# underdoc-wang/ST-MGCN

Hardware: AMD Instinct MI355X
Metric: train_samples_per_sec (higher is better)
Workload: dtype bf16; 1 GPU; model=ST_MGCN, preset=bench-1024, n_nodes=1024, seq_len=8, m_graphs=3, lstm_hidden=64, gcn_hidden=64, global_batch=32, parallelism=dp1, hipgraph=True, impl=hip

## Files before the change

### stmgcn_amd/csrc/fused_rnn.hip

```cpp

#include "common.h"

#define RNN_H 64
static_assert(4 * RNN_H == STM_DA_GATES, "dA tile layout assumes 4H = 256");
#define MAX_LAYERS 8
#define MAX_T 16

struct RnnPtrs {
  const void* w_ih[MAX_LAYERS];
  const void* w_hh[MAX_LAYERS];
  const void* b_ih[MAX_LAYERS];
  const void* b_hh[MAX_LAYERS];
};


extern "C" __global__ void mfma_probe_kernel(const __hip_bfloat16* A,
                                             const __hip_bfloat16* B, float* D) {
  const int l = threadIdx.x;
  bf16x8 a, b;
  #pragma unroll
      for (int j = 0; j < 8; ++j) {
    a[j] = *(const __bf16*)&A[(l % 16) * 32 + (l / 16) * 8 + j];
    b[j] = *(const __bf16*)&B[((l / 16) * 8 + j) * 16 + (l % 16)];
  }
  f32x4 c = {0.f, 0.f, 0.f, 0.f};
  c = mfma16x16x32(a, b, c);
  #pragma unroll
      for (int r = 0; r < 4; ++r) D[((l / 16) * 4 + r) * 16 + (l % 16)] = c[r];
}

template <typename F> __device__ __forceinline__ void rnn_uniform_bool(bool flag, F&& f) {
  if (flag) f(std::true_type{});
  else f(std::false_type{});
}

template <typename T, bool CIN1, bool GRU>
__global__ void __launch_bounds__(256, 2)
lstm_fwd_kernel(const T* __restrict__ x,
                T* __restrict__ out,
                T* __restrict__ hseq_g,
                T* __restrict__ cseq_g,
                T* __restrict__ gates_g,
                RnnPtrs ptrs,
                int S, int Tst, int L, int ret_seq) {
  using frag = typename Frag8<T>::type;
  using elem = typename Frag8<T>::elem;
  typedef elem elem4 __attribute__((ext_vector_type(4)));
  constexpr int MT = SEQ_TILE / 16;
  constexpr int SLOT = SEQ_TILE * 128;
  extern __shared__ char lds[];
  const int s0 = blockIdx.x * SEQ_TILE;
  const int wv = threadIdx.x >> 6;
  const int lane = threadIdx.x & 63;
  const int l16 = lane & 15;
  const int lgrp = lane >> 4;
  const long S_pad = (long)gridDim.x * SEQ_TILE;

  auto hslot = [&](int par) -> char* { return lds + (par & 1) * SLOT; };
  char* xbuf = lds + 2 * SLOT;

  if (CIN1) {
    for (int i = threadIdx.x; i < SEQ_TILE * Tst; i += 256) {
      const int s = i % SEQ_TILE, t = i / SEQ_TILE;
      T v = fromF<T>(0.f);
      if (s0 + s < S) v = x[(long)(s0 + s) * Tst + t];
      ((T*)xbuf)[t * SEQ_TILE + s] = v;
    }
    __syncthreads();
  }

  const int hch = 16 * wv + l16;
  const unsigned wlane = (hch * RNN_H + lgrp * 8) * sizeof(T);
  const unsigned inlane = (l16 * RNN_H + lgrp * 8) * sizeof(T);
  const unsigned savelane = (wv * MT * 64 + lane) * sizeof(T);

  auto layer_body = [&](int layer, auto first_c, auto train_c, auto top_c) {
    constexpr bool FIRST = decltype(first_c)::value;
    constexpr bool TRAIN = decltype(train_c)::value;
    constexpr bool TOP = decltype(top_c)::value;
    constexpr bool SCALAR = CIN1 && FIRST;
    constexpr bool KEEP_H = TRAIN || !TOP;
    const char* Whh = (const char*)ptrs.w_hh[layer];
    const char* Wih = (const char*)ptrs.w_ih[layer];
    const T* bih = (const T*)ptrs.b_ih[layer];
    const T* bhh = (const T*)ptrs.b_hh[layer];

    const T* hin = FIRST ? nullptr
        : hseq_g + ((long)(layer - 1) * Tst) * (S_pad * RNN_H) + (long)s0 * RNN_H;

    frag xfr[MT][2];
    auto load_input = [&](int t) {
      #pragma unroll
      for (int m = 0; m < MT; ++m) {
        #pragma unroll
        for (int kk = 0; kk < 2; ++kk) {
          if constexpr (FIRST) {
            const char* xt = (const char*)(x + ((long)(s0 + 16 * m) * Tst + t) * RNN_H);
            const unsigned xlane = (l16 * Tst * RNN_H + lgrp * 8) * sizeof(T);
            xfr[m][kk] = frag{};
            if (s0 + 16 * m + l16 < S)
              xfr[m][kk] = *(const frag*)(xt + (xlane + kk * 32 * sizeof(T)));
          } else {
            const char* ht = (const char*)(hin + (long)t * (S_pad * RNN_H));
            xfr[m][kk] = *(const frag*)(ht + (inlane + (m * 16 * RNN_H + kk * 32) * sizeof(T)));
          }
        }
      }
    };
    if constexpr (!SCALAR) load_input(0);

    frag bhfrag[4][2];
    #pragma unroll
    for (int q = 0; q < 4; ++q)
      #pragma unroll
      for (int kk = 0; kk < 2; ++kk)
        bhfrag[q][kk] = *(const frag*)(Whh + (wlane + (q * 64 * RNN_H + kk * 32) * sizeof(T)));
    frag bxfrag[4][2];
    if constexpr (!SCALAR) {
      #pragma unroll
      for (int q = 0; q < 4; ++q)
        #pragma unroll
        for (int kk = 0; kk < 2; ++kk)
          bxfrag[q][kk] = *(const frag*)(Wih + (wlane + (q * 64 * RNN_H + kk * 32) * sizeof(T)));
    }
    float wih0[4];
    float bias[4];
    #pragma unroll
    for (int q = 0; q < 4; ++q) {
      const int g = q * 64 + hch;
      bias[q] = toF<T>(bih[g]) + toF<T>(bhh[g]);
      if constexpr (SCALAR) wih0[q] = toF<T>(((const T*)Wih)[g]);
    }

    float c_state[MT][4];
    #pragma unroll
    for (int m = 0; m < MT; ++m)
      #pragma unroll
      for (int r = 0; r < 4; ++r) c_state[m][r] = 0.f;

    #pragma clang loop unroll(disable)
    for (int t = 0; t < Tst; ++t) {
      f32x4 acc[MT][4];
      const f32x4 zero4 = {0.f, 0.f, 0.f, 0.f};

      if (t > 0) {
        char* slot = hslot(t - 1);
        #pragma unroll
        for (int m = 0; m < MT; ++m) {
          const int row = 16 * m + l16;
          #pragma unroll
          for (int kk = 0; kk < 2; ++kk) {
            frag a = *(const frag*)&slot[lds_swz(row, (kk * 32 + lgrp * 8) * 2)];
            #pragma unroll
            for (int q = 0; q < 4; ++q)
              acc[m][q] = mfma16x16x32(a, bhfrag[q][kk], kk == 0 ? zero4 : acc[m][q]);
          }
        }
      } else {
        asm volatile("");
        #pragma unroll
        for (int m = 0; m < MT; ++m)
          #pragma unroll
          for (int q = 0; q < 4; ++q) acc[m][q] = zero4;
      }
      if constexpr (!SCALAR) {
        #pragma unroll
        for (int m = 0; m < MT; ++m)
          #pragma unroll
          for (int kk = 0; kk < 2; ++kk)
            #pragma unroll
            for (int q = 0; q < 4; ++q)
              acc[m][q] = mfma16x16x32(xfr[m][kk], bxfrag[q][kk], acc[m][q]);
        if (t + 1 < Tst) load_input(t + 1);
      }

      constexpr bool GRU_FUSED_ZH = CIN1 && std::is_same<T, __half>::value;
      T hval[MT][4];
      frag gsave[MT][2];
      elem4 csave[MT];
      #pragma unroll
      for (int m = 0; m < MT; ++m) {
        float xv[4];
        if constexpr (SCALAR) {
          #pragma unroll
          for (int r = 0; r < 4; ++r)
            xv[r] = toF<T>(((const T*)xbuf)[t * SEQ_TILE + 16 * m + 4 * lgrp + r]);
        }
        #pragma unroll
        for (int r = 0; r < 4; ++r) {
          float pre[4];
          #pragma unroll
          for (int q = 0; q < 4; ++q) {
            pre[q] = stm_fadd(acc[m][q][r], bias[q]);
            if constexpr (SCALAR) pre[q] = stm_fadd(pre[q], stm_fmul(xv[r], wih0[q]));
          }
          const float gi = pre[0], gf = pre[1], gg = pre[2], go = pre[3];
          if constexpr (GRU) {
            const float r_ = stm_sigmoid(gi), z_ = stm_sigmoid(gf);
            const float n_ = stm_tanh(fmaf(r_, go, gg));
            const float hprev = c_state[m][r];
            csave[m][r] = (elem)hprev;
            const float zn = stm_fmul(1.f - z_, n_);
            const float h_ = GRU_FUSED_ZH ? fmaf(z_, hprev, zn)
                                          : fmaf(1.f - z_, n_, stm_fmul(z_, hprev));
            c_state[m][r] = h_;
            if constexpr (GRU_FUSED_ZH) {
              unsigned hw;
              asm("v_fma_mixlo_f16 %0, %1, %2, %3"
                  : "=v"(hw) : "v"(hprev), "v"(z_), "v"(zn));
              hval[m][r] = __builtin_bit_cast(T, (unsigned short)hw);
            } else {
              hval[m][r] = fromF<T>(h_);
            }
            gsave[m][0][0 + r] = (elem)r_;
            gsave[m][0][4 + r] = (elem)z_;
            gsave[m][1][0 + r] = (elem)n_;
            gsave[m][1][4 + r] = (elem)go;
          } else {
            const float i_ = stm_sigmoid(gi), f_ = stm_sigmoid(gf);
            const float g_ = stm_tanh(gg), o_ = stm_sigmoid(go);
            const float ig = stm_fmul(i_, g_);
            const float c_ = CIN1 ? stm_fadd(stm_fmul(f_, c_state[m][r]), ig)
                                  : fmaf(f_, c_state[m][r], ig);
            c_state[m][r] = c_;
            csave[m][r] = (elem)c_;
            const float h_ = stm_fmul(o_, stm_tanh(c_));
            hval[m][r] = fromF<T>(h_);
            gsave[m][0][0 + r] = (elem)i_;
            gsave[m][0][4 + r] = (elem)f_;
            gsave[m][1][0 + r] = (elem)g_;
            gsave[m][1][4 + r] = (elem)o_;
          }
        }
      }

      {
        char* slot = hslot(t);
        #pragma unroll
        for (int m = 0; m < MT; ++m)
          #pragma unroll
          for (int r = 0; r < 4; ++r) {
            const int row = 16 * m + 4 * lgrp + r;
            *(T*)&slot[lds_swz(row, hch * 2)] = hval[m][r];
          }
      }
      __syncthreads();

      {
        static_assert(SEQ_TILE * 8 == 256, "one 16 B piece of the slot per thread");
        const int c8 = threadIdx.x & 7, sr = threadIdx.x >> 3;
        const frag v = *(const frag*)&hslot(t)[lds_swz(sr, c8 * 16)];
        if constexpr (KEEP_H) {
          char* hp = (char*)(hseq_g + ((long)layer * Tst + t) * (S_pad * RNN_H)
                             + (long)s0 * RNN_H);
          *(frag*)(hp + threadIdx.x * 16) = v;
        }
        if constexpr (TOP) {
          if (s0 + sr < S) {
            if (ret_seq)
              *(frag*)&out[((long)(s0 + sr) * Tst + t) * RNN_H + c8 * 8] = v;
            else if (t == Tst - 1)
              *(frag*)&out[(long)(s0 + sr) * RNN_H + c8 * 8] = v;
          }
        }
      }

      if constexpr (TRAIN) {
        const long base = ((long)layer * Tst + t);
        char* gp = (char*)(gates_g + base * (S_pad * 4 * RNN_H)
                           + (long)blockIdx.x * (SEQ_TILE * 4 * RNN_H));
        #pragma unroll
        for (int m = 0; m < MT; ++m)
          #pragma unroll
          for (int hq = 0; hq < 2; ++hq)
            *(frag*)(gp + (savelane * 16 + (m * 64 * 16 + hq * 8) * sizeof(T))) = gsave[m][hq];
        char* cp = (char*)(cseq_g + base * (S_pad * RNN_H)
                           + (long)blockIdx.x * (SEQ_TILE * RNN_H));
        #pragma unroll
        for (int m = 0; m < MT; ++m)
          *(elem4*)(cp + (savelane * 4 + m * 64 * 4 * sizeof(T))) = csave[m];
      }
    }
  };

  for (int layer = 0; layer < L; ++layer) {
    rnn_uniform_bool(layer == 0, [&](auto first_c) {
      rnn_uniform_bool(gates_g != nullptr, [&](auto train_c) {
        rnn_uniform_bool(layer == L - 1, [&](auto top_c) {
          layer_body(layer, first_c, train_c, top_c);
        });
      });
    });
    __threadfence_block();
    __syncthreads();
  }
}

static RnnPtrs rnn_ptrs(int L, const void** w_ih, const void** w_hh,
                        const void** b_ih, const void** b_hh) {
  RnnPtrs p{};
  for (int l = 0; l < L && l < MAX_LAYERS; ++l) {
    p.w_ih[l] = w_ih[l]; p.w_hh[l] = w_hh[l];
    p.b_ih[l] = b_ih ? b_ih[l] : nullptr;
    p.b_hh[l] = b_hh ? b_hh[l] : nullptr;
  }
  return p;
}

template <typename F> void rnn_dispatch_variant(int cin, int gru, F&& f) {
  stm_dispatch_bool(cin == 1, [&](auto cin1) {
    stm_dispatch_bool(gru != 0, [&](auto is_gru) { f(cin1, is_gru); });
  });
}

extern "C" void stmgcn_lstm_fwd(void* stream, int dtype, const void* x,
                                void* out, void* hseq_g, void* cseq_g,
                                void* gates_g, const void** w_ih,
                                const void** w_hh, const void** b_ih,
                                const void** b_hh, int S, int Tst, int L,
                                int cin, int ret_seq, int gru) {
  const RnnPtrs p = rnn_ptrs(L, w_ih, w_hh, b_ih, b_hh);
  const int nblk = (S + SEQ_TILE - 1) / SEQ_TILE;
  stm_dispatch_lowp("stmgcn_lstm_fwd", dtype, [&](auto t) {
    using T = decltype(t);
    const size_t lds_bytes =
        2 * SEQ_TILE * 128 + (cin == 1 ? Tst * SEQ_TILE * sizeof(T) : 0);
    rnn_dispatch_variant(cin, gru, [&](auto cin1, auto is_gru) {
      hipLaunchKernelGGL(
          (lstm_fwd_kernel<T, decltype(cin1)::value, decltype(is_gru)::value>),
          dim3(nblk), dim3(256), lds_bytes, (hipStream_t)stream, (const T*)x,
          (T*)out, (T*)hseq_g, (T*)cseq_g, (T*)gates_g, p, S, Tst, L, ret_seq);
    });
  });
}

extern "C" void stmgcn_mfma_probe(void* stream_v, const void* A, const void* B,
                                  void* D) {
  hipLaunchKernelGGL(mfma_probe_kernel, dim3(1), dim3(64), 0,
                     (hipStream_t)stream_v, (const __hip_bfloat16*)A,
                     (const __hip_bfloat16*)B, (float*)D);
}


template <typename T> __device__ __forceinline__ unsigned long pack4_word(f32x4 v) {
  unsigned long w = 0;
  #pragma unroll
  for (int r = 0; r < 4; ++r)
    w |= (unsigned long)__builtin_bit_cast(unsigned short, fromF<T>(v[r])) << (16 * r);
  return w;
}

template <int CTRL> __device__ __forceinline__ float dpp_row_add(float v) {
  return v + __int_as_float(__builtin_amdgcn_update_dpp(
                 0, __float_as_int(v), CTRL, 0xf, 0xf, false));
}

__device__ __forceinline__ int swzA(int s, int cbyte) {
  return s * 512 + (cbyte ^ ((s & 15) << 4));
}

template <typename T, bool CIN1, bool GRU>
__global__ void __launch_bounds__(256, 2)
lstm_bwd_kernel(const T* __restrict__ dout,
                const T* __restrict__ x,
                const T* __restrict__ cseq_g,
                const T* __restrict__ gates_g,
                RnnPtrs w,
                T* __restrict__ dx,
                T* __restrict__ dA_g,
                T* __restrict__ dh_g,
                int S, int Tst, int L, int ret_seq) {
  using frag = typename Frag8<T>::type;
  using elem = typename Frag8<T>::elem;
  constexpr int MT = SEQ_TILE / 16;
  extern __shared__ char lds[];
  const int s0 = blockIdx.x * SEQ_TILE;
  const int wv = threadIdx.x >> 6;
  const int lane = threadIdx.x & 63;
  const int l16 = lane & 15;
  const int lgrp = lane >> 4;
  const long S_pad = (long)gridDim.x * SEQ_TILE;
  const int hch = 16 * wv + l16;

  char* dA_lds = lds;
  float* red = (float*)(dA_lds + SEQ_TILE * 512);
  char* gstage = (char*)(red + 4 * SEQ_TILE);
  char* dhstage = gstage + 256 * (MT * 32);
  char* cstage = dhstage + 256 * (MT * 8);
  char* wstage = cstage + 2 * 256 * (MT * 8);
  char* wmine = wstage + threadIdx.x * 16;

  for (int layer = L - 1; layer >= 0; --layer) {
    const bool l0cin1 = CIN1 && layer == 0;
    const T* WhhT = (const T*)w.w_hh[layer];
    const T* WihT = (const T*)w.w_ih[layer];
    float dh_rec[MT][4], dc[MT][4];
    #pragma unroll
    for (int m = 0; m < MT; ++m)
      #pragma unroll
      for (int r = 0; r < 4; ++r) { dh_rec[m][r] = 0.f; dc[m][r] = 0.f; }

    const long lay_base = (long)layer * Tst;
    auto lane_frag = [&](int m) -> unsigned { return (wv * MT + m) * 64 + lane; };
    auto g_at = [&](int t) {
      return gates_g + (lay_base + t) * (S_pad * 4 * RNN_H)
             + (long)blockIdx.x * (SEQ_TILE * 4 * RNN_H);
    };
    auto c_at = [&](int t) {
      return cseq_g + (lay_base + t) * (S_pad * RNN_H)
             + (long)blockIdx.x * (SEQ_TILE * RNN_H);
    };
    auto dh_at = [&](int t) {
      return dh_g + (long)t * (S_pad * RNN_H)
             + (long)blockIdx.x * (SEQ_TILE * RNN_H);
    };
    char* gmine = gstage + threadIdx.x * (MT * 32);
    #pragma unroll
    for (int m = 0; m < MT; ++m) {
      *(frag*)&gmine[m * 32 + 0] =
          *(((const frag*)(g_at(Tst - 1) + lane_frag(m) * 16)) + 0);
      *(frag*)&gmine[m * 32 + 16] =
          *(((const frag*)(g_at(Tst - 1) + lane_frag(m) * 16)) + 1);
    }
    ulong1* dhmine = (ulong1*)(dhstage + threadIdx.x * (MT * 8));
    auto cmine = [&](int t) {
      return (ulong1*)(cstage + ((t & 1) * 256 + threadIdx.x) * (MT * 8));
    };
    if (layer < L - 1) {
      #pragma unroll
      for (int m = 0; m < MT; ++m)
        dhmine[m] = *(const ulong1*)(dh_at(Tst - 1) + lane_frag(m) * 4);
    }
    #pragma unroll
    for (int m = 0; m < MT; ++m) {
      cmine(Tst - 1)[m] = *(const ulong1*)(c_at(Tst - 1) + lane_frag(m) * 4);
      if (!GRU && Tst >= 2)
        cmine(Tst - 2)[m] = *(const ulong1*)(c_at(Tst - 2) + lane_frag(m) * 4);
    }
    {
      const unsigned wl = (hch * (4 * RNN_H) + lgrp * 8) * sizeof(T);
      #pragma unroll
      for (int kk = 0; kk < 8; ++kk)
        *(frag*)&wmine[kk * 4096] = *(const frag*)((const char*)WhhT + (wl + kk * 64));
    }
    float wih0[4];
    if (l0cin1) {
      #pragma unroll
      for (int q = 0; q < 4; ++q) wih0[q] = toF<T>(WihT[q * 64 + hch]);
    }
    __threadfence_block();
    __syncthreads();

    unsigned long dh_sent[MT] = {};
    #pragma clang loop unroll(disable)
    for (int t = Tst - 1;; --t) {
      const long base = lay_base + t;

      float dxpart[MT][4];
      alignas(16) T pk[4][MT * 4];

      const bool top_dout = layer == L - 1 && (ret_seq || t == Tst - 1);
      T dov[MT][4];
      if (top_dout) {
        const int dstride = ret_seq ? Tst * RNN_H : RNN_H;
        const T* dtile = dout + (long)s0 * dstride + (ret_seq ? t * RNN_H : 0);
        const int last = S - 1 - s0;
        int row0 = 4 * lgrp;
        asm volatile("" : "+v"(row0));
        #pragma unroll
        for (int m = 0; m < MT; ++m)
          #pragma unroll
          for (int r = 0; r < 4; ++r) {
            const int row = 16 * m + row0 + r;
            dov[m][r] = dtile[(row < last ? row : last) * dstride + hch];
          }
      }

      #pragma unroll
      for (int m = 0; m < MT; ++m) {
        frag gf0 = *(const frag*)&gmine[m * 32 + 0];
        frag gf1 = *(const frag*)&gmine[m * 32 + 16];
        const ulong1 cc_t = cmine(t)[m];
        const ulong1 cc_p = (!GRU && t > 0) ? cmine(t - 1)[m] : ulong1{0};
        ulong1 dhup = ulong1{0};
        if (layer < L - 1) dhup = dhmine[m];
        f32x4 ct, cpv;
        #pragma unroll
        for (int r = 0; r < 4; ++r) {
          ct[r] = elemF(((const elem*)&cc_t)[r]);
          cpv[r] = elemF(((const elem*)&cc_p)[r]);
        }
        #pragma unroll
        for (int r = 0; r < 4; ++r) {
          const int row = 16 * m + 4 * lgrp + r;
          float dh = dh_rec[m][r];
          if (layer < L - 1) {
            dh += elemF(((const elem*)&dhup)[r]);
          } else if (top_dout) {
            dh = (s0 + row < S) ? dh + toF<T>(dov[m][r]) : dh;
          }
          float dAi, dAf, dAg, dAo;
          if (GRU) {
            const float r_ = elemF(gf0[r]);
            const float z_ = elemF(gf0[4 + r]);
            const float n_ = elemF(gf1[r]);
            const float Bn = elemF(gf1[4 + r]);
            const float hprev = ct[r];
            dh += dc[m][r];
            const float dz_pre = dh * (hprev - n_) * z_ * (1.f - z_);
            const float dn_pre = dh * (1.f - z_) * (1.f - n_ * n_);
            const float dBn = dn_pre * r_;
            const float dr_pre = dn_pre * Bn * r_ * (1.f - r_);
            dc[m][r] = dh * z_;
            dAi = dr_pre; dAf = dz_pre; dAg = dn_pre; dAo = dBn;
          } else {
            const float i_ = elemF(gf0[r]);
            const float f_ = elemF(gf0[4 + r]);
            const float g_ = elemF(gf1[r]);
            const float o_ = elemF(gf1[4 + r]);
            const float tc = stm_tanh(ct[r]);
            float dcv = dc[m][r] + dh * o_ * (1.f - tc * tc);
            dAo = dh * tc * o_ * (1.f - o_);
            dAi = dcv * g_ * i_ * (1.f - i_);
            dAf = dcv * cpv[r] * f_ * (1.f - f_);
            dAg = dcv * i_ * (1.f - g_ * g_);
            dc[m][r] = dcv * f_;
          }
          pk[0][4 * m + r] = fromF<T>(dAi);
          pk[1][4 * m + r] = fromF<T>(dAf);
          pk[2][4 * m + r] = fromF<T>(dAg);
          pk[3][4 * m + r] = fromF<T>(dAo);
          #pragma unroll
          for (int q = 0; q < 4; ++q)
            *(T*)&dA_lds[swzA(row, (q * 64 + hch) * 2)] = pk[q][4 * m + r];
          if (l0cin1)
            dxpart[m][r] = dAi * wih0[0] + dAf * wih0[1] + dAg * wih0[2] + dAo * wih0[3];
        }
      }
      if (l0cin1) {
        #pragma unroll
        for (int m = 0; m < MT; ++m)
          #pragma unroll
          for (int r = 0; r < 4; ++r) dxpart[m][r] = dpp_row_add<0xB1>(dxpart[m][r]);
        #pragma unroll
        for (int m = 0; m < MT; ++m)
          #pragma unroll
          for (int r = 0; r < 4; ++r) dxpart[m][r] = dpp_row_add<0x4E>(dxpart[m][r]);
        #pragma unroll
        for (int m = 0; m < MT; ++m)
          #pragma unroll
          for (int r = 0; r < 4; ++r) dxpart[m][r] = dpp_row_add<0x141>(dxpart[m][r]);
        #pragma unroll
        for (int m = 0; m < MT; ++m)
          #pragma unroll
          for (int r = 0; r < 4; ++r) {
            const float v = dpp_row_add<0x140>(dxpart[m][r]);
            if (l16 == 0) red[wv * SEQ_TILE + 16 * m + 4 * lgrp + r] = v;
          }
      }
      T* out_dA = dA_g + stm_da_tile_off(base * S_pad + s0);
      #pragma unroll
      for (int q = 0; q < 4; ++q) *(frag*)&gmine[q * 16] = *(const frag*)pk[q];
      auto stage_rest = [&](auto rec_c, auto inp_c, auto up_c) {
        constexpr bool REC = decltype(rec_c)::value;
        constexpr bool INP = decltype(inp_c)::value;
        constexpr bool UP = decltype(up_c)::value;
        const unsigned wlane = (hch * (4 * RNN_H) + lgrp * 8) * sizeof(T);
        frag b2[2][4];
        f32x4 acc1[MT], acc2[MT];
        #pragma unroll
        for (int m = 0; m < MT; ++m) {
          acc1[m] = f32x4{0.f, 0.f, 0.f, 0.f};
          acc2[m] = f32x4{0.f, 0.f, 0.f, 0.f};
        }
        auto mfma_half = [&](int h) {
          frag b1[4];
          if constexpr (REC) {
            #pragma unroll
            for (int j = 0; j < 4; ++j) b1[j] = *(const frag*)&wmine[(4 * h + j) * 4096];
          }
          if constexpr (REC || INP) {
            #pragma unroll
            for (int jb = 0; jb < 4; jb += 2) {
              frag a[2][MT];
              #pragma unroll
              for (int j = 0; j < 2; ++j)
                #pragma unroll
                for (int m = 0; m < MT; ++m)
                  a[j][m] = *(const frag*)&dA_lds[swzA(16 * m + l16, ((4 * h + jb + j) * 32 + lgrp * 8) * 2)];
              #pragma unroll
              for (int j = 0; j < 2; ++j)
                #pragma unroll
                for (int m = 0; m < MT; ++m) {
                  if constexpr (REC) acc1[m] = mfma16x16x32(a[j][m], b1[jb + j], acc1[m]);
                  if constexpr (INP) acc2[m] = mfma16x16x32(a[j][m], b2[h][jb + j], acc2[m]);
                }
            }
          }
        };
        if constexpr (INP) {
          #pragma unroll
          for (int m = 0; m < MT; ++m) asm volatile("" :: "v"(dh_sent[m]));
        }
        if constexpr (INP) {
          #pragma unroll
          for (int kk = 0; kk < 8; ++kk)
            b2[kk / 4][kk % 4] = *(const frag*)((const char*)WihT + (wlane + kk * 64));
        }
        ulong1 dhnext[MT], cnext[MT];
        frag gld[MT][2];
        if constexpr (REC) {
          __builtin_amdgcn_sched_barrier(0);
          #pragma unroll
          for (int m = 0; m < MT; ++m) {
            gld[m][0] = *(((const frag*)(g_at(t - 1) + lane_frag(m) * 16)) + 0);
            gld[m][1] = *(((const frag*)(g_at(t - 1) + lane_frag(m) * 16)) + 1);
          }
          const int tc = GRU ? t - 1 : (t >= 2 ? t - 2 : 0);
          #pragma unroll
          for (int m = 0; m < MT; ++m)
            cnext[m] = *(const ulong1*)(c_at(tc) + lane_frag(m) * 4);
          if constexpr (UP) {
            #pragma unroll
            for (int m = 0; m < MT; ++m)
              dhnext[m] = *(const ulong1*)(dh_at(t - 1) + lane_frag(m) * 4);
          }
          __builtin_amdgcn_sched_barrier(0);
        }
        #pragma unroll
        for (int q = 0; q < 4; ++q)
          *(frag*)&out_dA[(unsigned)stm_da_elem(q * RNN_H + hch, 8 * lgrp)] =
              *(const frag*)&gmine[q * 16];

        __builtin_amdgcn_sched_barrier(0);
        __syncthreads();
        mfma_half(0);
        mfma_half(1);
        if constexpr (REC) {
          #pragma unroll
          for (int m = 0; m < MT; ++m)
            #pragma unroll
            for (int r = 0; r < 4; ++r) dh_rec[m][r] = acc1[m][r];
        }

        if constexpr (INP) {
          if (layer > 0) {
            #pragma unroll
            for (int m = 0; m < MT; ++m) {
              dh_sent[m] = pack4_word<T>(acc2[m]);
              *(unsigned long*)(dh_at(t) + lane_frag(m) * 4) = dh_sent[m];
            }
          } else {
            T* dxtile = dx + ((long)s0 * Tst + t) * RNN_H;
            const unsigned dxlane = 4 * lgrp * (Tst * RNN_H) + hch;
            #pragma unroll
            for (int m = 0; m < MT; ++m)
              #pragma unroll
              for (int r = 0; r < 4; ++r) {
                const int row = 16 * m + 4 * lgrp + r;
                if (s0 + row < S)
                  (dxtile + (16 * m + r) * (Tst * RNN_H))[dxlane] = fromF<T>(acc2[m][r]);
              }
          }
        } else {
          if (wv == 0) {
            for (int sA = lane; sA < SEQ_TILE; sA += 64) {
              const float v = red[sA] + red[SEQ_TILE + sA] + red[2 * SEQ_TILE + sA] + red[3 * SEQ_TILE + sA];
              if (s0 + sA < S) dx[(long)(s0 + sA) * Tst + t] = fromF<T>(v);
            }
          }
        }

        if constexpr (REC) {
          #pragma unroll
          for (int m = 0; m < MT; ++m) {
            *(frag*)&gmine[m * 32 + 0] = gld[m][0];
            *(frag*)&gmine[m * 32 + 16] = gld[m][1];
            cmine(GRU ? t - 1 : t)[m] = cnext[m];
            if constexpr (UP) dhmine[m] = dhnext[m];
          }
          __syncthreads();
        }
      };
      auto stage_rest_for = [&](auto rec_c) {
        rnn_uniform_bool(!l0cin1, [&](auto inp_c) {
          rnn_uniform_bool(layer < L - 1, [&](auto up_c) {
            stage_rest(rec_c, inp_c, up_c);
          });
        });
      };
      if (t == 0) {
        stage_rest_for(std::false_type{});
        break;
      }
      stage_rest_for(std::true_type{});
    }
  }
}

extern "C" void stmgcn_lstm_bwd(void* stream, int dtype, const void* dout,
                                const void* x, const void* cseq_g,
                                const void* gates_g, const void** w_ihT,
                                const void** w_hhT, void* dx, void* dA_g,
                                void* dh_g, int S, int Tst, int L, int cin,
                                int ret_seq, int gru) {
  const RnnPtrs p = rnn_ptrs(L, w_ihT, w_hhT, nullptr, nullptr);
  const int nblk = (S + SEQ_TILE - 1) / SEQ_TILE;
  const size_t lds_bytes = SEQ_TILE * 512 + 4 * SEQ_TILE * sizeof(float)
                           + 256 * (SEQ_TILE / 16) * (32 + 3 * 8)
                           + RNN_H * 4 * RNN_H * 2;
  stm_dispatch_lowp("stmgcn_lstm_bwd", dtype, [&](auto t) {
    using T = decltype(t);
    rnn_dispatch_variant(cin, gru, [&](auto cin1, auto is_gru) {
      STM_CHECK_HIP(hipFuncSetAttribute(
          (const void*)lstm_bwd_kernel<T, decltype(cin1)::value, decltype(is_gru)::value>,
          hipFuncAttributeMaxDynamicSharedMemorySize, (int)lds_bytes));
      hipLaunchKernelGGL(
          (lstm_bwd_kernel<T, decltype(cin1)::value, decltype(is_gru)::value>),
          dim3(nblk), dim3(256), lds_bytes, (hipStream_t)stream, (const T*)dout,
          (const T*)x, (const T*)cseq_g, (const T*)gates_g, p, (T*)dx,
          (T*)dA_g, (T*)dh_g, S, Tst, L, ret_seq);
    });
  });
}

struct PackMats {
  const unsigned short* src[2 * MAX_LAYERS];
  long dst_off[2 * MAX_LAYERS];
  int cols[2 * MAX_LAYERS];
};

__global__ void __launch_bounds__(256)
lstm_pack_bwd_weights_kernel(PackMats pm, unsigned short* __restrict__ dst) {
  __shared__ unsigned short tile[64][66];
  const unsigned short* src = pm.src[blockIdx.y];
  unsigned short* out = dst + pm.dst_off[blockIdx.y];
  const int cols = pm.cols[blockIdx.y];
  const int r0 = blockIdx.x * 64;
  const int lo = threadIdx.x & 63, hi = threadIdx.x >> 6;
  for (int r = hi; r < 64; r += 4)
    if (lo < cols) tile[r][lo] = src[(long)(r0 + r) * cols + lo];
  __syncthreads();
  for (int c = hi; c < cols; c += 4)
    out[(long)c * 256 + r0 + lo] = tile[lo][c];
}

extern "C" void stmgcn_lstm_pack_bwd_weights(void* stream, const void** w_ih,
                                             const void** w_hh, int L, int cin,
                                             void* dst) {
  PackMats pm{};
  long off = 0;
  for (int l = 0; l < L && l < MAX_LAYERS; ++l) {
    pm.src[l] = (const unsigned short*)w_ih[l];
    pm.cols[l] = l == 0 ? cin : 64;
    pm.dst_off[l] = off;
    off += 256L * pm.cols[l];
  }
  for (int l = 0; l < L && l < MAX_LAYERS; ++l) {
    pm.src[L + l] = (const unsigned short*)w_hh[l];
    pm.cols[L + l] = 64;
    pm.dst_off[L + l] = off;
    off += 256L * 64;
  }
  hipLaunchKernelGGL(lstm_pack_bwd_weights_kernel, dim3(4, 2 * L), dim3(256), 0,
                     (hipStream_t)stream, pm, (unsigned short*)dst);
}
```

Measured before the change: 14350 samples/s.

## Restructure LSTM backward: transposed dA LDS layout, per-layer template specialization

After: 15000 samples/s, median of 6. 4.5% higher.

```diff
diff --git a/stmgcn_amd/csrc/fused_rnn.hip b/stmgcn_amd/csrc/fused_rnn.hip
--- a/stmgcn_amd/csrc/fused_rnn.hip
+++ b/stmgcn_amd/csrc/fused_rnn.hip
@@ -352,11 +352,21 @@
 
 template <int CTRL> __device__ __forceinline__ float dpp_row_add(float v) {
   return v + __int_as_float(__builtin_amdgcn_update_dpp(
-                 0, __float_as_int(v), CTRL, 0xf, 0xf, false));
-}
-
-__device__ __forceinline__ int swzA(int s, int cbyte) {
-  return s * 512 + (cbyte ^ ((s & 15) << 4));
+                 0, __float_as_int(v), CTRL, 0xf, 0xf, true));
+}
+
+__device__ __forceinline__ int dA_img(int c, int slot) {
+  return c * 64 + ((slot ^ ((c >> 1) & 7)) << 3);
+}
+
+template <typename T> __device__ __forceinline__ T stm_fmul_to(float a, float b) {
+  if constexpr (std::is_same<T, __half>::value) {
+    unsigned hw;
+    asm("v_fma_mixlo_f16 %0, %1, %2, 0" : "=v"(hw) : "v"(a), "v"(b));
+    return __builtin_bit_cast(T, (unsigned short)hw);
+  } else {
+    return fromF<T>(stm_fmul(a, b));
+  }
 }
 
 template <typename T, bool CIN1, bool GRU>
@@ -390,8 +400,19 @@
   char* wstage = cstage + 2 * 256 * (MT * 8);
   char* wmine = wstage + threadIdx.x * 16;
 
-  for (int layer = L - 1; layer >= 0; --layer) {
-    const bool l0cin1 = CIN1 && layer == 0;
+  int dA_wr[MT], dA_rd[2][MT];
+  #pragma unroll
+  for (int m = 0; m < MT; ++m) {
+    dA_wr[m] = dA_img(hch, 4 * m + lgrp);
+    #pragma unroll
+    for (int hf = 0; hf < 2; ++hf)
+      dA_rd[hf][m] = dA_img(8 * lgrp + 4 * hf + (l16 >> 2), 4 * m + (l16 & 3));
+  }
+
+  constexpr int DH_UP = 0, DH_SEQ = 1, DH_LAST = 2;
+  auto layer_body = [&](int layer, auto scalar_c, auto src_c) {
+    constexpr bool SCALAR = CIN1 && decltype(scalar_c)::value;
+    constexpr int SRC = decltype(src_c)::value;
     const T* WhhT = (const T*)w.w_hh[layer];
     const T* WihT = (const T*)w.w_ih[layer];
     float dh_rec[MT][4], dc[MT][4];
@@ -399,6 +420,37 @@
     for (int m = 0; m < MT; ++m)
       #pragma unroll
       for (int r = 0; r < 4; ++r) { dh_rec[m][r] = 0.f; dc[m][r] = 0.f; }
+
+    auto load_dout = [&](const T* dtile, int dstride, T (&dov)[MT][4]) {
+      const int last = S - 1 - s0;
+      #pragma unroll
+      for (int m = 0; m < MT; ++m)
+        #pragma unroll
+        for (int r = 0; r < 4; ++r) {
+          const int row = 16 * m + 4 * lgrp + r;
+          dov[m][r] = dtile[(row < last ? row : last) * dstride + hch];
+        }
+    };
+    auto dout_f32 = [&](const T (&dov)[MT][4], float (&dof)[MT][4]) {
+      #pragma unroll
+      for (int m = 0; m < MT; ++m)
+        #pragma unroll
+        for (int r = 0; r < 4; ++r) dof[m][r] = toF<T>(dov[m][r]);
+      static_assert(MT == 2, "eight operands");
+      asm volatile("" : "+v"(dof[0][0]), "+v"(dof[0][1]), "+v"(dof[0][2]), "+v"(dof[0][3]),
+                        "+v"(dof[1][0]), "+v"(dof[1][1]), "+v"(dof[1][2]), "+v"(dof[1][3]));
+    };
+    if constexpr (SRC == DH_LAST) {
+      T dov[MT][4];
+      float dof[MT][4];
+      load_dout(dout + (long)s0 * RNN_H, RNN_H, dov);
+      dout_f32(dov, dof);
+      #pragma unroll
+      for (int m = 0; m < MT; ++m)
+        #pragma unroll
+        for (int r = 0; r < 4; ++r)
+          dh_rec[m][r] = (s0 + 16 * m + 4 * lgrp + r < S) ? stm_fadd(0.f, dof[m][r]) : 0.f;
+    }
 
     const long lay_base = (long)layer * Tst;
     auto lane_frag = [&](int m) -> unsigned { return (wv * MT + m) * 64 + lane; };
@@ -426,7 +478,7 @@
     auto cmine = [&](int t) {
       return (ulong1*)(cstage + ((t & 1) * 256 + threadIdx.x) * (MT * 8));
     };
-    if (layer < L - 1) {
+    if constexpr (SRC == DH_UP) {
       #pragma unroll
       for (int m = 0; m < MT; ++m)
         dhmine[m] = *(const ulong1*)(dh_at(Tst - 1) + lane_frag(m) * 4);
@@ -444,7 +496,7 @@
         *(frag*)&wmine[kk * 4096] = *(const frag*)((const char*)WhhT + (wl + kk * 64));
     }
     float wih0[4];
-    if (l0cin1) {
+    if constexpr (SCALAR) {
       #pragma unroll
       for (int q = 0; q < 4; ++q) wih0[q] = toF<T>(WihT[q * 64 + hch]);
     }
@@ -459,21 +511,11 @@
       float dxpart[MT][4];
       alignas(16) T pk[4][MT * 4];
 
-      const bool top_dout = layer == L - 1 && (ret_seq || t == Tst - 1);
-      T dov[MT][4];
-      if (top_dout) {
-        const int dstride = ret_seq ? Tst * RNN_H : RNN_H;
-        const T* dtile = dout + (long)s0 * dstride + (ret_seq ? t * RNN_H : 0);
-        const int last = S - 1 - s0;
-        int row0 = 4 * lgrp;
-        asm volatile("" : "+v"(row0));
-        #pragma unroll
-        for (int m = 0; m < MT; ++m)
-          #pragma unroll
-          for (int r = 0; r < 4; ++r) {
-            const int row = 16 * m + row0 + r;
-            dov[m][r] = dtile[(row < last ? row : last) * dstride + hch];
-          }
+      float dof[MT][4];
+      if constexpr (SRC == DH_SEQ) {
+        T dov[MT][4];
+        load_dout(dout + ((long)s0 * Tst + t) * RNN_H, Tst * RNN_H, dov);
+        dout_f32(dov, dof);
       }
 
       #pragma unroll
@@ -481,9 +523,13 @@
         frag gf0 = *(const frag*)&gmine[m * 32 + 0];
         frag gf1 = *(const frag*)&gmine[m * 32 + 16];
         const ulong1 cc_t = cmine(t)[m];
-        const ulong1 cc_p = (!GRU && t > 0) ? cmine(t - 1)[m] : ulong1{0};
+        ulong1 cc_p = ulong1{0};
+        if constexpr (!GRU) {
+          cc_p = cmine(t - 1)[m];
+          cc_p = t > 0 ? cc_p : ulong1{0};
+        }
         ulong1 dhup = ulong1{0};
-        if (layer < L - 1) dhup = dhmine[m];
+        if constexpr (SRC == DH_UP) dhup = dhmine[m];
         f32x4 ct, cpv;
         #pragma unroll
         for (int r = 0; r < 4; ++r) {
@@ -494,50 +540,53 @@
         for (int r = 0; r < 4; ++r) {
           const int row = 16 * m + 4 * lgrp + r;
           float dh = dh_rec[m][r];
-          if (layer < L - 1) {
-            dh += elemF(((const elem*)&dhup)[r]);
-          } else if (top_dout) {
-            dh = (s0 + row < S) ? dh + toF<T>(dov[m][r]) : dh;
-          }
-          float dAi, dAf, dAg, dAo;
-          if (GRU) {
+          if constexpr (SRC == DH_UP) {
+            dh = stm_fadd(dh, elemF(((const elem*)&dhup)[r]));
+          } else if constexpr (SRC == DH_SEQ) {
+            dh = (s0 + row < S) ? stm_fadd(dh, dof[m][r]) : dh;
+          }
+          float fa[4], fb[4];
+          if constexpr (GRU) {
             const float r_ = elemF(gf0[r]);
             const float z_ = elemF(gf0[4 + r]);
             const float n_ = elemF(gf1[r]);
             const float Bn = elemF(gf1[4 + r]);
             const float hprev = ct[r];
-            dh += dc[m][r];
-            const float dz_pre = dh * (hprev - n_) * z_ * (1.f - z_);
-            const float dn_pre = dh * (1.f - z_) * (1.f - n_ * n_);
-            const float dBn = dn_pre * r_;
-            const float dr_pre = dn_pre * Bn * r_ * (1.f - r_);
-            dc[m][r] = dh * z_;
-            dAi = dr_pre; dAf = dz_pre; dAg = dn_pre; dAo = dBn;
+            dh = stm_fadd(dh, dc[m][r]);
+            const float dnp = stm_fmul(dh, 1.f - z_);
+            const float dnq = 1.f - stm_fmul(n_, n_);
+            const float dn_pre = stm_fmul(dnp, dnq);
+            fa[0] = stm_fmul(stm_fmul(dn_pre, Bn), r_); fb[0] = 1.f - r_;
+            fa[1] = stm_fmul(stm_fmul(dh, hprev - n_), z_); fb[1] = 1.f - z_;
+            fa[2] = dnp; fb[2] = dnq;
+            fa[3] = dn_pre; fb[3] = r_;
+            dc[m][r] = stm_fmul(dh, z_);
           } else {
             const float i_ = elemF(gf0[r]);
             const float f_ = elemF(gf0[4 + r]);
             const float g_ = elemF(gf1[r]);
             const float o_ = elemF(gf1[4 + r]);
             const float tc = stm_tanh(ct[r]);
-            float dcv = dc[m][r] + dh * o_ * (1.f - tc * tc);
-            dAo = dh * tc * o_ * (1.f - o_);
-            dAi = dcv * g_ * i_ * (1.f - i_);
-            dAf = dcv * cpv[r] * f_ * (1.f - f_);
-            dAg = dcv * i_ * (1.f - g_ * g_);
-            dc[m][r] = dcv * f_;
-          }
-          pk[0][4 * m + r] = fromF<T>(dAi);
-          pk[1][4 * m + r] = fromF<T>(dAf);
-          pk[2][4 * m + r] = fromF<T>(dAg);
-          pk[3][4 * m + r] = fromF<T>(dAo);
-          #pragma unroll
-          for (int q = 0; q < 4; ++q)
-            *(T*)&dA_lds[swzA(row, (q * 64 + hch) * 2)] = pk[q][4 * m + r];
-          if (l0cin1)
-            dxpart[m][r] = dAi * wih0[0] + dAf * wih0[1] + dAg * wih0[2] + dAo * wih0[3];
-        }
-      }
-      if (l0cin1) {
+            const float dcv = fmaf(stm_fmul(dh, o_), 1.f - stm_fmul(tc, tc), dc[m][r]);
+            fa[0] = stm_fmul(stm_fmul(dcv, g_), i_); fb[0] = 1.f - i_;
+            fa[1] = stm_fmul(stm_fmul(dcv, cpv[r]), f_); fb[1] = 1.f - f_;
+            fa[2] = stm_fmul(dcv, i_); fb[2] = 1.f - stm_fmul(g_, g_);
+            fa[3] = stm_fmul(stm_fmul(dh, tc), o_); fb[3] = 1.f - o_;
+            dc[m][r] = stm_fmul(dcv, f_);
+          }
+          #pragma unroll
+          for (int q = 0; q < 4; ++q) pk[q][4 * m + r] = stm_fmul_to<T>(fa[q], fb[q]);
+          if constexpr (SCALAR)
+            dxpart[m][r] = fmaf(stm_fmul(fa[3], fb[3]), wih0[3],
+                           fmaf(stm_fmul(fa[2], fb[2]), wih0[2],
+                           fmaf(stm_fmul(fa[0], fb[0]), wih0[0],
+                                stm_fmul(stm_fmul(fa[1], fb[1]), wih0[1]))));
+        }
+        #pragma unroll
+        for (int q = 0; q < 4; ++q)
+          *(unsigned long*)&dA_lds[q * 4096 + dA_wr[m]] = *(const unsigned long*)&pk[q][4 * m];
+      }
+      if constexpr (SCALAR) {
         #pragma unroll
         for (int m = 0; m < MT; ++m)
           #pragma unroll
@@ -553,18 +602,21 @@
         #pragma unroll
         for (int m = 0; m < MT; ++m)
           #pragma unroll
-          for (int r = 0; r < 4; ++r) {
-            const float v = dpp_row_add<0x140>(dxpart[m][r]);
-            if (l16 == 0) red[wv * SEQ_TILE + 16 * m + 4 * lgrp + r] = v;
-          }
+          for (int r = 0; r < 4; ++r) dxpart[m][r] = dpp_row_add<0x140>(dxpart[m][r]);
+        if (l16 == 0) {
+          #pragma unroll
+          for (int m = 0; m < MT; ++m)
+            *(f32x4*)&red[wv * SEQ_TILE + 16 * m + 4 * lgrp] =
+                f32x4{dxpart[m][0], dxpart[m][1], dxpart[m][2], dxpart[m][3]};
+        }
       }
       T* out_dA = dA_g + stm_da_tile_off(base * S_pad + s0);
       #pragma unroll
       for (int q = 0; q < 4; ++q) *(frag*)&gmine[q * 16] = *(const frag*)pk[q];
-      auto stage_rest = [&](auto rec_c, auto inp_c, auto up_c) {
+      auto stage_rest = [&](auto rec_c) {
         constexpr bool REC = decltype(rec_c)::value;
-        constexpr bool INP = decltype(inp_c)::value;
-        constexpr bool UP = decltype(up_c)::value;
+        constexpr bool INP = !SCALAR;
+        constexpr bool UP = SRC == DH_UP;
         const unsigned wlane = (hch * (4 * RNN_H) + lgrp * 8) * sizeof(T);
         frag b2[2][4];
         f32x4 acc1[MT], acc2[MT];
@@ -586,8 +638,16 @@
               #pragma unroll
               for (int j = 0; j < 2; ++j)
                 #pragma unroll
-                for (int m = 0; m < MT; ++m)
-                  a[j][m] = *(const frag*)&dA_lds[swzA(16 * m + l16, ((4 * h + jb + j) * 32 + lgrp * 8) * 2)];
+                for (int m = 0; m < MT; ++m) {
+                  typedef short short4v __attribute__((ext_vector_type(4)));
+                  typedef short short8v __attribute__((ext_vector_type(8)));
+                  typedef __attribute__((address_space(3))) short4v* lds_s4;
+                  const char* p = dA_lds + (4 * h + jb + j) * 2048;
+                  const short4v lo = __builtin_amdgcn_ds_read_tr16_b64_v4i16((lds_s4)(p + dA_rd[0][m]));
+                  const short4v hi = __builtin_amdgcn_ds_read_tr16_b64_v4i16((lds_s4)(p + dA_rd[1][m]));
+                  a[j][m] = __builtin_bit_cast(
+                      frag, __builtin_shufflevector(lo, hi, 0, 1, 2, 3, 4, 5, 6, 7));
+                }
               #pragma unroll
               for (int j = 0; j < 2; ++j)
                 #pragma unroll
@@ -682,19 +742,25 @@
           __syncthreads();
         }
       };
-      auto stage_rest_for = [&](auto rec_c) {
-        rnn_uniform_bool(!l0cin1, [&](auto inp_c) {
-          rnn_uniform_bool(layer < L - 1, [&](auto up_c) {
-            stage_rest(rec_c, inp_c, up_c);
-          });
+      if (t == 0) {
+        stage_rest(std::false_type{});
+        break;
+      }
+      stage_rest(std::true_type{});
+    }
+  };
+
+  for (int layer = L - 1; layer >= 0; --layer) {
+    rnn_uniform_bool(CIN1 && layer == 0, [&](auto scalar_c) {
+      if (layer < L - 1) {
+        layer_body(layer, scalar_c, std::integral_constant<int, DH_UP>{});
+      } else {
+        rnn_uniform_bool(ret_seq != 0, [&](auto seq_c) {
+          layer_body(layer, scalar_c,
+                     std::integral_constant<int, decltype(seq_c)::value ? DH_SEQ : DH_LAST>{});
         });
-      };
-      if (t == 0) {
-        stage_rest_for(std::false_type{});
-        break;
-      }
-      stage_rest_for(std::true_type{});
-    }
+      }
+    });
   }
 }
 
```
